# gnovack/distributed-training-and-deepspeed

Hardware: AMD Instinct MI355X
Metric: tokens/sec (whole node) BERT-base DDP (higher is better)
Workload: dtype bf16; 1 GPU; model=bert-base-cased, params=108340804, global_batch=1024, per_gpu_batch=1024, seq_len=512, parallelism=dp1, grad_dtype=bfloat16, impl=fused, mlm_head=sparse (labelled rows only, static capacity 80896; identical loss/grads), optimizer=fused AdamW (transformers.AdamW hyper-params, lr 5e-5), tuned_gemms=True, hip_graph=False, force_collectives=False, prewarm=auto, async_wgrad=False, opt_overlap=True

## Files before the change

distributed_training_and_deepspeed_amd/ops/csrc/attention.hip:

```cpp
#include <stdio.h>
#include <type_traits>
#include <stdlib.h>
#include <string.h>

#include "common.h"

#ifndef DTD_ATTN_FUSED_BWD
#define DTD_ATTN_FUSED_BWD 0
#endif

using namespace dtd;

typedef float f32x16 __attribute__((ext_vector_type(16)));

namespace {

constexpr float kLog2e = 1.4426950408889634f;
constexpr float kLn2 = 0.6931471805599453f;

typedef short s16x4 __attribute__((ext_vector_type(4)));
typedef __attribute__((address_space(3))) s16x4 lds_s16x4;

__device__ __forceinline__ f32x16 mfma32(bf16x8 a, bf16x8 b, f32x16 c) {
  return __builtin_amdgcn_mfma_f32_32x32x16_bf16(a, b, c, 0, 0, 0);
// ... 37 lines not shown
}
__device__ __forceinline__ float keep_bits(float v, uint32_t w, int b) {
  return __int_as_float(__float_as_int(v) & bit_mask(w, b));
}

__device__ __forceinline__ float xhalf_max(float x) {
  const auto r = __builtin_amdgcn_permlane32_swap(__float_as_uint(x), __float_as_uint(x), false, false);
  return fmaxf(__uint_as_float(r[0]), __uint_as_float(r[1]));
}
__device__ __forceinline__ float xhalf_sum(float x) {
  const auto r = __builtin_amdgcn_permlane32_swap(__float_as_uint(x), __float_as_uint(x), false, false);
  return __uint_as_float(r[0]) + __uint_as_float(r[1]);
}
__device__ __forceinline__ uint32_t half_word(uint32_t w, int hh) { return w >> (4 * hh); }
constexpr float kRescaleThr = 8.f;

typedef float f32x2 __attribute__((ext_vector_type(2)));
__device__ __forceinline__ f32x2 pk_fma(f32x2 a, f32x2 b, f32x2 c) { return __builtin_elementwise_fma(a, b, c); }
__device__ __forceinline__ f32x2 pk2(float x, float y) { return f32x2{x, y}; }
__device__ __forceinline__ float mask_bits(float v, int m) { return __int_as_float(__float_as_int(v) & m); }

__device__ __forceinline__ int lm_pos(int x) {
  const int c = x & 31;
  return (x & ~31) | (c & 24) | ((c & 3) << 1) | ((c >> 2) & 1);
}
__device__ __forceinline__ float sel_keep(float v, uint64_t m) {
  float r;
  asm("v_cndmask_b32_e64 %0, 0, %1, %2" : "=v"(r) : "v"(v), "s"(m));
  return r;
}
typedef __attribute__((address_space(4))) const uint64_t cu64;
__device__ __forceinline__ int keep_off(int off, int Sp) { return min(off, Sp - 32); }

struct FwdArgs {
  const bf16* q; const bf16* k; const bf16* v; bf16* o; float* lse; const float* slopes;
  const uint32_t* maskA;
  const uint32_t* maskB;
  int B, S, H, ld, ldo, causal, W;
  float scale, p, thr;
  const int* kv_range;
};

__device__ __forceinline__ void load_range(const int* kv_range, int b, int S, int& lo, int& hi) {
  lo = __builtin_amdgcn_readfirstlane(min(max(kv_range[2 * b], 0), S));
  hi = __builtin_amdgcn_readfirstlane(max(min(kv_range[2 * b + 1], S), 0));
}

template <int S_>
__device__ __forceinline__ uint32_t swap_stage(uint32_t t, uint32_t sh, uint32_t mk) {
  const uint32_t y = (uint32_t)__builtin_amdgcn_ds_swizzle((int)t, (S_ << 10) | 0x1f);
  const uint32_t rot = __builtin_amdgcn_alignbit(y, y, sh);
  return (rot & mk) | (t & ~mk);
}
constexpr int kMaskRot = 13;
__global__ void __launch_bounds__(256) attn_mask_kernel(uint32_t* __restrict__ maskA, uint32_t* __restrict__ maskB,
                                                        int S, int W, const uint64_t* rng, uint32_t sid, uint32_t thr) {
  const int lane = threadIdx.x & 63, bh = blockIdx.y;
  const int q0 = blockIdx.x * 256 + (threadIdx.x & ~63);
  if (q0 >= 32 * W) return;
  DropoutRng g(rng, sid);
  const int q = q0 + lane;
  const bool qv = q < S;
  uint32_t st[16];
  {
    uint32_t x = g.bits((uint64_t)bh * S + (uint64_t)(qv ? q : 0));
    x = x ? x : 0x6d2b79f5u;
#pragma unroll
    for (int i = 0; i < 16; ++i) {
      if (i) { x ^= x << 13; x ^= x >> 17; x ^= x << 5; }
      st[i] = x;
    }
  }
  uint32_t nt[16];
#pragma unroll
  for (int i = 0; i < 16; ++i) nt[i] = ((thr >> i) & 1u) ? 0u : 0xffffffffu;
  const uint32_t live = (qv && thr < 65536u) ? 0xffffffffu : 0u;
  uint32_t sh[5], mk[5];
#pragma unroll
  for (int i = 0; i < 5; ++i) {
    const int s = 16 >> i;
    const uint32_t Hs = i == 0 ? 0xffff0000u : i == 1 ? 0xff00ff00u : i == 2 ? 0xf0f0f0f0u : i == 3 ? 0xccccccccu : 0xaaaaaaaau;
    const bool up = lane & s;
    sh[i] = up ? s : 32 - s;
    mk[i] = up ? ~Hs : Hs;
  }
  const int qw = q0 / 32 + (lane >> 5);
  uint32_t* pa = maskA + (size_t)bh * W * (32 * W) + lm_pos(q);
  for (int kw = 0; kw < W; ++kw) {
    uint32_t acc = 0xffffffffu;
#pragma unroll
    for (int i = 0; i < 16; ++i) {
      st[i] += __builtin_amdgcn_alignbit(st[(i + 11) & 15], st[(i + 11) & 15], 32 - kMaskRot);
      acc = __builtin_amdgcn_bitop3_b32(st[i], acc, nt[i], 0xe8);
    }
    uint32_t word = acc & live;
    const int nk = S - kw * 32;
    if (nk < 32) word &= (0xffffffffu >> (32 - nk));
    if (qv) pa[(size_t)kw * (32 * W)] = word;
    uint32_t t = word;
    t = swap_stage<16>(t, sh[0], mk[0]);
    t = swap_stage<8>(t, sh[1], mk[1]);
    t = swap_stage<4>(t, sh[2], mk[2]);
    t = swap_stage<2>(t, sh[3], mk[3]);
    t = swap_stage<1>(t, sh[4], mk[4]);
    const int key = kw * 32 + (lane & 31);
    if (key < S && qw < W) maskB[((size_t)bh * W + qw) * (32 * W) + lm_pos(key)] = t;
  }
}

__device__ __forceinline__ void xcd_tile(int& tx, int& ty) {
  const int nx = gridDim.x, n = nx * gridDim.y;
  const int L = blockIdx.x + nx * blockIdx.y;
  if (n % 8) { tx = blockIdx.x; ty = blockIdx.y; return; }
  const int T = (L % 8) * (n / 8) + L / 8;
  tx = T % nx;
  ty = T / nx;
}

__device__ __forceinline__ void xcd_tile_grouped(int& tx, int& ty) {
  constexpr int kGroup = 32;
  const int nx = gridDim.x, n = nx * gridDim.y;
  const int L = blockIdx.x + nx * blockIdx.y;
  if (n % 8) { tx = blockIdx.x; ty = blockIdx.y; return; }
  const int per = n / 8, gs = kGroup * nx;
  int i = L / 8;
  if (i < (per / gs) * gs) {
    const int r = i % gs;
    i = (i - r) + (r % kGroup) * nx + r / kGroup;
  }
  const int T = (L % 8) * per + i;
  tx = T % nx;
  ty = T / nx;
}

__device__ __forceinline__ __amdgpu_buffer_rsrc_t bounded_rsrc(const void* p, uint32_t bytes) {
  const uint64_t a = (uint64_t)p;
  const uint32_t lo = __builtin_amdgcn_readfirstlane((uint32_t)a);
  const uint32_t hi = __builtin_amdgcn_readfirstlane((uint32_t)(a >> 32));
  return __builtin_amdgcn_make_buffer_rsrc((void*)(((uint64_t)hi << 32) | lo), (short)0, (int)bytes, 0x00020000);
}

struct RowSrc {
  __amdgpu_buffer_rsrc_t rs;
  int voff, ld2;
};
template <int D>
__device__ __forceinline__ RowSrc row_src(const bf16* base, int ld, int nrows) {
  RowSrc r;
  r.rs = bounded_rsrc(base, nrows > 0 ? (uint32_t)(((nrows - 1) * ld + D) * 2) : 0u);
  r.voff = ((threadIdx.x / (D / 8)) * ld + (threadIdx.x % (D / 8)) * 8) * 2;
  r.ld2 = ld * 2;
  return r;
}
struct WordSrc {
  __amdgpu_buffer_rsrc_t rs;
  int voff, stride;
  __device__ __forceinline__ uint32_t load(int wi) const {
    return __builtin_amdgcn_raw_buffer_load_b32(rs, voff, wi * stride, 0);
  }
};
__device__ __forceinline__ WordSrc word_src(const uint32_t* words, const void* dummy, int W, int pos) {
  WordSrc w;
  const int Sp = 32 * W;
  w.rs = bounded_rsrc(words ? (const void*)words : dummy, words ? (uint32_t)W * Sp * 4u : 0u);
  w.voff = lm_pos(pos) * 4;
  w.stride = Sp * 4;
  return w;
}

template <int D, int ROWS>
struct TileLoader {
  static constexpr int CH = ROWS * D / 8;
  static constexpr int PER = (CH + 255) / 256;
  static constexpr int RPI = 256 / (D / 8);
  bf16x8 reg[PER];
  static_assert(CH % 256 == 0, "tile must split evenly over 256 threads");
  __device__ __forceinline__ void load(const RowSrc& src, int row0) {
#pragma unroll
    for (int i = 0; i < PER; ++i)
      reg[i] = __builtin_bit_cast(bf16x8, __builtin_amdgcn_raw_buffer_load_b128(src.rs, src.voff, (row0 + RPI * i) * src.ld2, 0));
  }
  __device__ __forceinline__ void store(bf16* lds, int stride) const {
#pragma unroll
    for (int i = 0; i < PER; ++i) {
      const int c = threadIdx.x + 256 * i;
      *reinterpret_cast<bf16x8*>(lds + (c / (D / 8)) * stride + (c % (D / 8)) * 8) = reg[i];
    }
  }
  __device__ __forceinline__ void store_swz(bf16* lds) const {
    static_assert(D == 64, "swizzled tile image is for 64-column tiles");
#pragma unroll
    for (int i = 0; i < PER; ++i) {
      const int c = threadIdx.x + 256 * i;
      *reinterpret_cast<bf16x8*>(lds + swz64_off(c >> 3, c & 7)) = reg[i];
    }
  }
  __device__ __forceinline__ void store_bwd(bf16* lds, int stride) const {
    if constexpr (D == 64) store_swz(lds);
    else store(lds, stride);
  }
};

template <int D, int OCC, int BN, int RING, bool PK = false, bool RANGE = false>
__global__ void __launch_bounds__(256, OCC) attn_fwd_kernel(FwdArgs a) {
  constexpr int KP = D + 8, VP = D + 32, NC = D / 16, NDB = D / 32, NKB = BN / 32;
  __shared__ __attribute__((aligned(16))) bf16 Ks[2][BN * KP];
  __shared__ __attribute__((aligned(16))) bf16 Vs[2][BN * VP];

  const int lane = threadIdx.x & 63, w = __builtin_amdgcn_readfirstlane(threadIdx.x >> 6), hh = lane >> 5,
            r = lane & 31;
  int tx, ty;
  xcd_tile(tx, ty);
  const int bh = ty, b = bh / a.H, h = bh % a.H;
  const int S = a.S;
  const int qblk = tx * 128, q0 = qblk + w * 32;
  const int q = q0 + r;
  const bool qvalid = q < S;
  const float sl2 = a.slopes ? a.slopes[h] * kLog2e : 0.f;
  const float sc2 = a.scale * kLog2e;
  const bool drop = a.maskA != nullptr;
  const float inv_keep = drop ? 1.f / (1.f - a.p) : 1.f;
  const RowSrc ksrc = row_src<D>(a.k + (size_t)b * S * a.ld + h * D, a.ld, S);
  const RowSrc vsrc = row_src<D>(a.v + (size_t)b * S * a.ld + h * D, a.ld, S);
  const int Sp = 32 * a.W;
  const uint32_t* mrow = drop ? a.maskB + ((size_t)bh * a.W + min(q0 >> 5, a.W - 1)) * Sp : nullptr;
  const __amdgpu_buffer_rsrc_t mrs = bounded_rsrc(drop ? (const void*)mrow : (const void*)a.lse, drop ? (uint32_t)Sp * 4u : 0u);

  bf16x8 qf[NC];
  {
    const bf16* qp = a.q + ((size_t)(b * S + (qvalid ? q : 0)) * a.ld + h * D);
#pragma unroll
    for (int c = 0; c < NC; ++c) qf[c] = qvalid ? *reinterpret_cast<const bf16x8*>(qp + 16 * c + 8 * hh) : bf16x8{};
  }
  f32x16 oacc[NDB];
#pragma unroll
  for (int d = 0; d < NDB; ++d) oacc[d] = f32x16{};
  float m = -INFINITY, l = 0.f;

  int klo = 0, khi = S;
  if constexpr (RANGE) load_range(a.kv_range, b, S, klo, khi);
  const int kend = a.causal ? min(khi, qblk + 128) : khi;
  const int nt = (kend + BN - 1) / BN;
  const int t0 = RANGE ? klo / BN : 0;
  const int last = RANGE ? max(nt - 1, t0) : nt - 1;
  TileLoader<D, BN> kl0, vl0, kl1r, vl1r;
  TileLoader<D, BN>& kl1 = RING == 2 ? kl1r : kl0;
  TileLoader<D, BN>& vl1 = RING == 2 ? vl1r : vl0;
  uint32_t pf0 = 0, pf1r = 0;
  uint32_t& pf1 = RING == 2 ? pf1r : pf0;
  auto prefetch_words = [&](int k0, uint32_t& out) {
    asm volatile("" :: "v"(out));
    out = __builtin_amdgcn_raw_buffer_load_b32(mrs, lane * 4, k0 * 4, 0);
  };
  kl0.load(ksrc, t0 * BN);
  vl0.load(vsrc, t0 * BN);
  kl0.store(Ks[0], KP);
  vl0.store(Vs[0], VP);
  {
    const int k1 = min(t0 + 1, last) * BN, k2 = min(t0 + 2, last) * BN;
    kl1.load(ksrc, k1); vl1.load(vsrc, k1); prefetch_words(k1, pf1);
    if constexpr (RING == 2) { kl0.load(ksrc, k2); vl0.load(vsrc, k2); prefetch_words(k2, pf0); }
  }
  __syncthreads();
  auto tile = [&](auto set_c, int t) {
    constexpr int SET = decltype(set_c)::value;
    TileLoader<D, BN>& kn = SET ? kl1 : kl0;
    TileLoader<D, BN>& vn = SET ? vl1 : vl0;
    uint32_t& pfn = SET ? pf1 : pf0;
    const int buf = (t - t0) & 1, k0 = t * BN;
    const bf16* K = Ks[buf];
    const bf16* V = Vs[buf];
    uint64_t mk[16];
    auto load_masks = [&](int kb) {
      const cu64* mp = (const cu64*)(uintptr_t)(mrow + keep_off(k0 + kb * 32, Sp));
#pragma unroll
      for (int i = 0; i < 16; ++i) mk[i] = mp[i];
    };
    f32x16 sacc[NKB];
#pragma unroll
    for (int kb = 0; kb < NKB; ++kb) {
      f32x16 acc = f32x16{};
#pragma unroll
      for (int c = 0; c < NC; ++c)
        acc = mfma32(*reinterpret_cast<const bf16x8*>(&K[(kb * 32 + r) * KP + 16 * c + 8 * hh]), qf[c], acc);
      sacc[kb] = acc;
    }
    if (drop) load_masks(0);
    const bool needmask = (k0 + BN > khi) || (RANGE && k0 < klo) || (a.causal && k0 + BN - 1 > q0);
    const bool slow = needmask || sl2 != 0.f;
    float tmax = -INFINITY;
    if (slow) {
#pragma unroll
      for (int kb = 0; kb < NKB; ++kb)
#pragma unroll
        for (int i = 0; i < 16; ++i) {
          const int key = k0 + kb * 32 + crow(i, hh);
          float s = fmaf(sacc[kb][i], sc2, sl2 * (float)key);
          if (needmask && (key >= khi || (RANGE && key < klo) || (a.causal && key > q))) s = -INFINITY;
          sacc[kb][i] = s;
          tmax = fmaxf(tmax, s);
        }
    } else {
#pragma unroll
      for (int kb = 0; kb < NKB; ++kb)
#pragma unroll
        for (int i = 0; i < 16; ++i) tmax = fmaxf(tmax, sacc[kb][i]);
// ... 173 lines not shown
#pragma unroll
        for (int i = 0; i < 16; ++i) tmax = fmaxf(tmax, cur[kb][i]);
      tmax *= sc2;
    }
    tmax = xhalf_max(tmax);
    if (!__all(tmax - m <= a.thr)) {
      const float mnew = fmaxf(m, tmax);
      const float alpha = m == -INFINITY ? 0.f : fexp2(m - mnew);
      m = mnew;
      l *= alpha;
#pragma unroll
      for (int d = 0; d < NDB; ++d) oacc[d] *= alpha;
    }
    scores_kb(Knext, nxt, 1);
    const float mexp = m == -INFINITY ? 0.f : m;
    const float msc = slow ? 1.f : sc2;
    float ps[4];
#pragma unroll
    for (int kb = 0; kb < NKB; ++kb)
#pragma unroll
      for (int i = 0; i < 16; ++i) {
        const float pv = fexp2(fmaf(cur[kb][i], msc, -mexp));
        ps[i & 3] = (kb == 0 && i < 4) ? pv : ps[i & 3] + pv;
        cur[kb][i] = pv;
      }
    l += (ps[0] + ps[1]) + (ps[2] + ps[3]);
    if (drop) {
#pragma unroll
      for (int kb = 0; kb < NKB; ++kb) {
        const uint32_t mw = half_word(mwc[kb], hh);
#pragma unroll
        for (int i = 0; i < 16; ++i) cur[kb][i] = keep_bits(cur[kb][i], mw, crow(i, 0));
      }
    }
#pragma unroll
    for (int kb = 0; kb < NKB; ++kb)
#pragma unroll
      for (int s2 = 0; s2 < 2; ++s2) {
        bf16x8 pf;
#pragma unroll
        for (int j = 0; j < 8; ++j) pf[j] = (bf16)cur[kb][8 * s2 + j];
#pragma unroll
        for (int d = 0; d < NDB; ++d) oacc[d] = mfma32(tr_operand(V, VP, kb * 32 + 16 * s2, d * 32, lane), pf, oacc[d]);
      }
    if (t + 1 < nt) {
      if (t + 2 < nt) kl.store(Ks[t & 1], KP);
      vl.store(Vs[(t + 1) & 1], VP);
#pragma unroll
      for (int j = 0; j < NKB; ++j) mwc[j] = mwn[j];
      kl.load(ksrc, min(t + 3, last) * BN);
      vl.load(vsrc, min(t + 2, last) * BN);
      load_words(min(t + 2, last) * BN, mwn);
    }
    __syncthreads();
  };
  f32x16 sA[NKB], sB[NKB];
#pragma unroll
  for (int kb = 0; kb < NKB; ++kb) scores_kb(Ks[0], sA, kb);
  for (int t = 0; t < nt; t += 2) {
    tile_step(sA, sB, Ks[1], t);
    if (t + 1 < nt) tile_step(sB, sA, Ks[0], t + 1);
  }
  l = xhalf_sum(l);
  if (!qvalid) return;
  const float inv_l = l > 0.f ? inv_keep / l : 0.f;
  bf16* op = a.o + (size_t)(b * S + q) * a.ldo + h * D;
#pragma unroll
  for (int d = 0; d < NDB; ++d)
#pragma unroll
    for (int gq = 0; gq < 4; ++gq) {
      bf16x4 v4;
#pragma unroll
      for (int t = 0; t < 4; ++t) v4[t] = (bf16)(oacc[d][4 * gq + t] * inv_l);
      *reinterpret_cast<bf16x4*>(op + d * 32 + 8 * gq + 4 * hh) = v4;
    }
  if (hh == 0) a.lse[(size_t)bh * S + q] = (m + log2f(l)) * kLn2;
}

struct BwdArgs {
  const bf16* q; const bf16* k; const bf16* v; const bf16* dout; const float* lse; float* delta;
  const bf16* o;
  bf16* dq; bf16* dk; bf16* dv; const float* slopes;
  const uint32_t* maskA; const uint32_t* maskB;
  int B, S, H, ld, ldo, causal, W;
  float scale, p;
  float* bias_part;
  const int* kv_range;
};

template <int S_>
__device__ __forceinline__ float xswz(float x) {
  return __int_as_float(__builtin_amdgcn_ds_swizzle(__float_as_int(x), (S_ << 10) | 0x1f));
}
template <int S_, int N>
__device__ __forceinline__ void rs_step(const float (&in)[2 * N], float (&out)[N], int r) {
  const bool hi = (r & S_) != 0;
#pragma unroll
  for (int j = 0; j < N; ++j) {
    const float mine = hi ? in[j + N] : in[j];
    const float other = hi ? in[j] : in[j + N];
    out[j] = mine + xswz<S_>(other);
  }
}
__device__ __forceinline__ float colsum32(const float (&v)[32], int r) {
  float a16[16], a8[8], a4[4], a2[2], a1[1];
  rs_step<16, 16>(v, a16, r);
  rs_step<8, 8>(a16, a8, r);
  rs_step<4, 4>(a8, a4, r);
  rs_step<2, 2>(a4, a2, r);
  rs_step<1, 1>(a2, a1, r);
  return a1[0];
}
__device__ __forceinline__ int colsum_col(int k, int hh) { return (k >> 4) * 32 + crow(k & 15, hh); }

template <int D, int OCC, int BM, bool DROP, bool ALIBI, bool MASK = true, bool RANGE = false>
__global__ void __launch_bounds__(256, OCC) attn_bwd_dkdv_kernel(BwdArgs a) {
  static_assert(MASK || !RANGE, "a key range needs the masked form");
  constexpr bool SWZ = D == 64;
  constexpr int QP = SWZ ? D : D + 8, NC = D / 16, NDB = D / 32;
  struct Smem {
    float lse_s[2][BM], del_s[2][BM];
    bf16 Qs[2][BM * QP];
    bf16 Os[2][BM * QP];
  };
  __shared__ __attribute__((aligned(16))) Smem sm;
  auto& lse_s = sm.lse_s;
  auto& del_s = sm.del_s;
  auto& Qs = sm.Qs;
  auto& Os = sm.Os;

  const int lane = threadIdx.x & 63, w = __builtin_amdgcn_readfirstlane(threadIdx.x >> 6), hh = lane >> 5,
            r = lane & 31;
  int tx, ty;
  if constexpr (RANGE) xcd_tile_grouped(tx, ty);
  else xcd_tile(tx, ty);
  const int bh = ty, b = bh / a.H, h = bh % a.H;
  const int S = a.S;
  const int kblk = tx * 128;
  const int key = kblk + w * 32 + r;
  const bool kvalid = key < S;
  int klo = 0, khi = S;
  if constexpr (RANGE) {
    load_range(a.kv_range, b, S, klo, khi);
    if (kblk >= khi || kblk + 128 <= klo) {
      if (a.bias_part && D == 64) {
        float* row = a.bias_part + ((size_t)b * gridDim.x * 4 + (kblk >> 5) + w) * (3 * a.H * D) + h * D + colsum_col(r, hh);
        row[a.H * D] = 0.f;
        row[2 * a.H * D] = 0.f;
      }
      if (kvalid) {
        bf16* dkp = a.dk + (size_t)(b * S + key) * a.ld + h * D;
        bf16* dvp = a.dv + (size_t)(b * S + key) * a.ld + h * D;
#pragma unroll
        for (int c = 0; c < D / 8; ++c) {
          *reinterpret_cast<bf16x4*>(dkp + 8 * c + 4 * hh) = bf16x4{};
          *reinterpret_cast<bf16x4*>(dvp + 8 * c + 4 * hh) = bf16x4{};
        }
      }
      return;
    }
  }
  const bool kin = key >= klo && key < khi;
  const float sl2 = a.slopes ? a.slopes[h] * kLog2e : 0.f;
  const float sc2 = a.scale * kLog2e;
  constexpr bool drop = DROP;
  const float inv_keep = drop ? 1.f / (1.f - a.p) : 1.f;
  const float kbias = sl2 * (float)key;
  const int Sp = 32 * a.W;
  const uint32_t* mrow = drop ? a.maskA + ((size_t)bh * a.W + min((kblk >> 5) + w, a.W - 1)) * Sp : nullptr;
  const __amdgpu_buffer_rsrc_t mrs = bounded_rsrc(drop ? (const void*)mrow : (const void*)a.lse, drop ? (uint32_t)Sp * 4u : 0u);
  const RowSrc qsrc = row_src<D>(a.q + (size_t)b * S * a.ld + h * D, a.ld, S);
  const RowSrc osrc = row_src<D>(a.dout + (size_t)b * S * a.ldo + h * D, a.ldo, S);
  const float* lseb = a.lse + (size_t)bh * S;
  const float* delb = a.delta + (size_t)bh * S;

  bf16x8 kf[NC], vf[NC];
  {
    const size_t off = (size_t)(b * S + (kvalid ? key : 0)) * a.ld + h * D;
#pragma unroll
    for (int c = 0; c < NC; ++c) {
      kf[c] = kvalid ? *reinterpret_cast<const bf16x8*>(a.k + off + 16 * c + 8 * hh) : bf16x8{};
      vf[c] = kvalid ? *reinterpret_cast<const bf16x8*>(a.v + off + 16 * c + 8 * hh) : bf16x8{};
    }
  }
  f32x16 dk[NDB], dv[NDB];
#pragma unroll
  for (int d = 0; d < NDB; ++d) { dk[d] = f32x16{}; dv[d] = f32x16{}; }

  const int qstart = a.causal ? (kblk / BM) * BM : 0;
  const int nt = (S - qstart + BM - 1) / BM;
  TileLoader<D, BM> ql, ol;
  float lse_r = 0.f, del_r = 0.f;
  auto load_stats = [&](int q0) {
    if (threadIdx.x < BM) {
      const int qq = q0 + threadIdx.x;
      lse_r = qq < S ? -lseb[qq] * kLog2e : 0.f;
      if constexpr (RANGE) lse_r = lse_r == INFINITY ? -INFINITY : lse_r;
      del_r = qq < S ? -delb[qq] * (DROP ? 1.f - a.p : 1.f) : 0.f;
    }
  };
  constexpr int NPF = BM / 64;
  uint32_t pfw[NPF] = {};
  auto prefetch_words = [&](int q0) {
#pragma unroll
    for (int j = 0; j < NPF; ++j) {
      asm volatile("" :: "v"(pfw[j]));
      pfw[j] = __builtin_amdgcn_raw_buffer_load_b32(mrs, (lane + 64 * j) * 4, q0 * 4, 0);
    }
  };
  ql.load(qsrc, qstart);
  ol.load(osrc, qstart);
  load_stats(qstart);
  ql.store_bwd(Qs[0], QP);
  ol.store_bwd(Os[0], QP);
  if (threadIdx.x < BM) { lse_s[0][threadIdx.x] = lse_r; del_s[0][threadIdx.x] = del_r; }
  __syncthreads();
  for (int t = 0; t < nt; ++t) {
    const int buf = t & 1, q0 = qstart + t * BM;
    if (t + 1 < nt) {
      ql.load(qsrc, q0 + BM);
      ol.load(osrc, q0 + BM);
      load_stats(q0 + BM);
      if (drop) prefetch_words(q0 + BM);
    }
    const bf16* Q = Qs[buf];
    const bf16* O = Os[buf];
    constexpr int kQbUnroll = OCC == 1 ? BM / 32 : 1;
#pragma unroll kQbUnroll
    for (int qb = 0; qb < BM / 32; ++qb) {
      f32x16 sacc = f32x16{}, pacc = f32x16{};
#pragma unroll
      for (int c = 0; c < NC; ++c) {
        if constexpr (SWZ) {
          sacc = mfma32(swz_row_read(Q, qb * 32, r, 2 * c + hh), kf[c], sacc);
          pacc = mfma32(swz_row_read(O, qb * 32, r, 2 * c + hh), vf[c], pacc);
        } else {
          sacc = mfma32(*reinterpret_cast<const bf16x8*>(&Q[(qb * 32 + r) * QP + 16 * c + 8 * hh]), kf[c], sacc);
          pacc = mfma32(*reinterpret_cast<const bf16x8*>(&O[(qb * 32 + r) * QP + 16 * c + 8 * hh]), vf[c], pacc);
        }
      }
      const int qrow0 = q0 + qb * 32;
      bool needmask = MASK && ((kblk + 128 > S) || (qrow0 + 32 > S) || (a.causal && kblk + 127 > qrow0));
      if constexpr (RANGE) needmask = needmask || kblk + 128 > khi || kblk < klo;
      uint64_t mk[16];
      if constexpr (DROP) {
        const cu64* mp = (const cu64*)(uintptr_t)(mrow + keep_off(qrow0, Sp));
#pragma unroll
        for (int i = 0; i < 16; ++i) mk[i] = mp[i];
      }
      f32x4 L4[4], D4[4];
#pragma unroll
      for (int g = 0; g < 4; ++g) {
        L4[g] = *reinterpret_cast<const f32x4*>(&lse_s[buf][qb * 32 + 8 * g + 4 * hh]);
        D4[g] = *reinterpret_cast<const f32x4*>(&del_s[buf][qb * 32 + 8 * g + 4 * hh]);
      }
      const f32x2 sc2v = pk2(sc2, sc2), kb2 = pk2(kbias, kbias);
#pragma unroll
      for (int i = 0; i < 16; i += 2) {
        f32x2 nl = pk2(L4[i >> 2][i & 3], L4[i >> 2][(i & 3) + 1]);
        if constexpr (ALIBI) nl += kb2;
        const f32x2 x = pk_fma(pk2(sacc[i], sacc[i + 1]), sc2v, nl);
        sacc[i] = fexp2(x.x);
        sacc[i + 1] = fexp2(x.y);
      }
      if (MASK && needmask) {
#pragma unroll
        for (int i = 0; i < 16; ++i) {
          const int qq = qrow0 + crow(i, hh);
          bool ok = kvalid && qq < S && !(a.causal && key > qq);
          if constexpr (RANGE) ok = ok && kin;
          sacc[i] = ok ? sacc[i] : 0.f;
        }
      }
#pragma unroll
      for (int i = 0; i < 16; i += 2) {
        const f32x2 nd = pk2(D4[i >> 2][i & 3], D4[i >> 2][(i & 3) + 1]);
        if constexpr (DROP) {
          const f32x2 pm = pk2(sel_keep(sacc[i], mk[i]), sel_keep(sacc[i + 1], mk[i + 1]));
          const f32x2 u = pk2(sacc[i], sacc[i + 1]) * nd;
          const f32x2 ds = pk_fma(pm, pk2(pacc[i], pacc[i + 1]), u);
          pacc[i] = ds.x;
          pacc[i + 1] = ds.y;
          sacc[i] = pm.x;
          sacc[i + 1] = pm.y;
        } else {
          const f32x2 ds = pk2(sacc[i], sacc[i + 1]) * (pk2(pacc[i], pacc[i + 1]) + nd);
          pacc[i] = ds.x;
          pacc[i + 1] = ds.y;
        }
      }
#pragma unroll
      for (int s = 0; s < 2; ++s) {
        bf16x8 pb, sb;
#pragma unroll
        for (int j = 0; j < 8; ++j) { pb[j] = (bf16)sacc[8 * s + j]; sb[j] = (bf16)pacc[8 * s + j]; }
#pragma unroll
        for (int d = 0; d < NDB; ++d) {
          if constexpr (SWZ) {
            dv[d] = mfma32(tr_operand_swz(O, qb * 32 + 16 * s, d * 32, lane), pb, dv[d]);
            dk[d] = mfma32(tr_operand_swz(Q, qb * 32 + 16 * s, d * 32, lane), sb, dk[d]);
          } else {
            dv[d] = mfma32(tr_operand(O, QP, qb * 32 + 16 * s, d * 32, lane), pb, dv[d]);
            dk[d] = mfma32(tr_operand(Q, QP, qb * 32 + 16 * s, d * 32, lane), sb, dk[d]);
          }
        }
      }
    }
    if (t + 1 < nt) {
      ql.store_bwd(Qs[buf ^ 1], QP);
      ol.store_bwd(Os[buf ^ 1], QP);
      if (threadIdx.x < BM) { lse_s[buf ^ 1][threadIdx.x] = lse_r; del_s[buf ^ 1][threadIdx.x] = del_r; }
    }
    __syncthreads();
  }
  const float dv_scale = inv_keep;
  const float dk_scale = a.scale * inv_keep;
  if (a.bias_part && D == 64) {
    float vk[32], vv[32];
#pragma unroll
    for (int d = 0; d < NDB; ++d)
#pragma unroll
      for (int i = 0; i < 16; ++i) {
        vk[16 * d + i] = kvalid ? (float)(bf16)(dk[d][i] * dk_scale) : 0.f;
        vv[16 * d + i] = kvalid ? (float)(bf16)(dv[d][i] * dv_scale) : 0.f;
      }
    const float sk = colsum32(vk, r), sv = colsum32(vv, r);
    float* row = a.bias_part + ((size_t)b * gridDim.x * 4 + (kblk >> 5) + w) * (3 * a.H * D) + h * D + colsum_col(r, hh);
    row[a.H * D] = sk;
    row[2 * a.H * D] = sv;
  }
  if (!kvalid) return;
  bf16* dkp = a.dk + (size_t)(b * S + key) * a.ld + h * D;
  bf16* dvp = a.dv + (size_t)(b * S + key) * a.ld + h * D;
#pragma unroll
  for (int d = 0; d < NDB; ++d)
#pragma unroll
    for (int gq = 0; gq < 4; ++gq) {
      bf16x4 k4, v4;
#pragma unroll
      for (int t = 0; t < 4; ++t) { k4[t] = (bf16)(dk[d][4 * gq + t] * dk_scale); v4[t] = (bf16)(dv[d][4 * gq + t] * dv_scale); }
      *reinterpret_cast<bf16x4*>(dkp + d * 32 + 8 * gq + 4 * hh) = k4;
      *reinterpret_cast<bf16x4*>(dvp + d * 32 + 8 * gq + 4 * hh) = v4;
    }
}

template <int D, int OCC, int BN, int RING, bool PK = false, bool RANGE = false>
__global__ void __launch_bounds__(256, OCC) attn_bwd_dq_kernel(BwdArgs a) {
  constexpr bool SWZ = D == 64;
  constexpr int KP = SWZ ? D : D + 8, NC = D / 16, NDB = D / 32;
  __shared__ __attribute__((aligned(16))) bf16 Ks[2][BN * KP];
  __shared__ __attribute__((aligned(16))) bf16 Vs[2][BN * KP];

  const int lane = threadIdx.x & 63, w = __builtin_amdgcn_readfirstlane(threadIdx.x >> 6), hh = lane >> 5,
            r = lane & 31;
  int tx, ty;
  xcd_tile(tx, ty);
  const int bh = ty, b = bh / a.H, h = bh % a.H;
  const int S = a.S;
  const int qblk = tx * 128, q0 = qblk + w * 32;
  const int q = q0 + r;
  const bool qvalid = q < S;
  const float sl2 = a.slopes ? a.slopes[h] * kLog2e : 0.f;
  const float sc2 = a.scale * kLog2e;
  const bool drop = a.maskA != nullptr;
  const float inv_keep = drop ? 1.f / (1.f - a.p) : 1.f;
  const RowSrc ksrc = row_src<D>(a.k + (size_t)b * S * a.ld + h * D, a.ld, S);
  const RowSrc vsrc = row_src<D>(a.v + (size_t)b * S * a.ld + h * D, a.ld, S);
  const int Sp = 32 * a.W;
  const uint32_t* mrow = drop ? a.maskB + ((size_t)bh * a.W + min(q0 >> 5, a.W - 1)) * Sp : nullptr;
  const __amdgpu_buffer_rsrc_t mrs = bounded_rsrc(drop ? (const void*)mrow : (const void*)a.lse, drop ? (uint32_t)Sp * 4u : 0u);

  bf16x8 qf[NC], of[NC];
  {
    const bf16* qp = a.q + ((size_t)(b * S + (qvalid ? q : 0)) * a.ld + h * D);
    const bf16* op = a.dout + ((size_t)(b * S + (qvalid ? q : 0)) * a.ldo + h * D);
#pragma unroll
    for (int c = 0; c < NC; ++c) {
      qf[c] = qvalid ? *reinterpret_cast<const bf16x8*>(qp + 16 * c + 8 * hh) : bf16x8{};
      of[c] = qvalid ? *reinterpret_cast<const bf16x8*>(op + 16 * c + 8 * hh) : bf16x8{};
    }
  }
  float lse2 = qvalid ? a.lse[(size_t)bh * S + q] * kLog2e : 0.f;
  if constexpr (RANGE) lse2 = lse2 == -INFINITY ? INFINITY : lse2;
  float dl;
  {
    const bf16* orow = a.o + ((size_t)(b * S + (qvalid ? q : 0)) * a.ldo + h * D);
    float part = 0.f;
#pragma unroll
    for (int c = 0; c < NC; ++c) {
      const bf16x8 ov = qvalid ? *reinterpret_cast<const bf16x8*>(orow + 16 * c + 8 * hh) : bf16x8{};
#pragma unroll
      for (int j = 0; j < 8; ++j) part = fmaf((float)ov[j], (float)of[c][j], part);
    }
    dl = xhalf_sum(part);
    if (qvalid && hh == 0) a.delta[(size_t)bh * S + q] = dl;
  }
  f32x16 dq[NDB];
#pragma unroll
  for (int d = 0; d < NDB; ++d) dq[d] = f32x16{};

  int klo = 0, khi = S;
  if constexpr (RANGE) load_range(a.kv_range, b, S, klo, khi);
  const int kend = a.causal ? min(khi, qblk + 128) : khi;
  const int nt = (kend + BN - 1) / BN;
  const int t0 = RANGE ? klo / BN : 0;
  const int last = RANGE ? max(nt - 1, t0) : nt - 1;
  constexpr int NKB = BN / 32;
  TileLoader<D, BN> kl0, vl0, kl1r, vl1r;
  TileLoader<D, BN>& kl1 = RING == 2 ? kl1r : kl0;
  TileLoader<D, BN>& vl1 = RING == 2 ? vl1r : vl0;
  uint32_t pf0 = 0, pf1r = 0;
  uint32_t& pf1 = RING == 2 ? pf1r : pf0;
  auto prefetch_words = [&](int k0, uint32_t& out) {
    asm volatile("" :: "v"(out));
    out = __builtin_amdgcn_raw_buffer_load_b32(mrs, lane * 4, k0 * 4, 0);
  };
  kl0.load(ksrc, t0 * BN);
  vl0.load(vsrc, t0 * BN);
  kl0.store_bwd(Ks[0], KP);
  vl0.store_bwd(Vs[0], KP);
  {
    const int k1 = min(t0 + 1, last) * BN, k2 = min(t0 + 2, last) * BN;
    kl1.load(ksrc, k1); vl1.load(vsrc, k1); prefetch_words(k1, pf1);
    if constexpr (RING == 2) { kl0.load(ksrc, k2); vl0.load(vsrc, k2); prefetch_words(k2, pf0); }
  }
  __syncthreads();
  auto tile = [&](auto set_c, int t) {
    constexpr int SET = decltype(set_c)::value;
    TileLoader<D, BN>& kn = SET ? kl1 : kl0;
    TileLoader<D, BN>& vn = SET ? vl1 : vl0;
    uint32_t& pfn = SET ? pf1 : pf0;
    const int buf = (t - t0) & 1, k0 = t * BN;
    const bf16* K = Ks[buf];
    const bf16* V = Vs[buf];
    const bool needmask = !qvalid || (k0 + BN > khi) || (RANGE && k0 < klo) || (a.causal && k0 + BN - 1 > q0);
#pragma unroll
    for (int kb = 0; kb < BN / 32; ++kb) {
      f32x16 sacc = f32x16{}, pacc = f32x16{};
#pragma unroll
      for (int c = 0; c < NC; ++c) {
        if constexpr (SWZ) {
          sacc = mfma32(swz_row_read(K, kb * 32, r, 2 * c + hh), qf[c], sacc);
          pacc = mfma32(swz_row_read(V, kb * 32, r, 2 * c + hh), of[c], pacc);
        } else {
          sacc = mfma32(*reinterpret_cast<const bf16x8*>(&K[(kb * 32 + r) * KP + 16 * c + 8 * hh]), qf[c], sacc);
          pacc = mfma32(*reinterpret_cast<const bf16x8*>(&V[(kb * 32 + r) * KP + 16 * c + 8 * hh]), of[c], pacc);
        }
      }
      uint64_t mk[16];
      if (drop) {
        const cu64* mp = (const cu64*)(uintptr_t)(mrow + keep_off(k0 + kb * 32, Sp));
#pragma unroll
        for (int i = 0; i < 16; ++i) mk[i] = mp[i];
      }
      if (needmask || sl2 != 0.f) {
#pragma unroll
        for (int i = 0; i < 16; ++i) {
          const int key = k0 + kb * 32 + crow(i, hh);
          float pv = fexp2(fmaf(sacc[i], sc2, sl2 * (float)key - lse2));
          if (needmask && (!qvalid || key >= khi || (RANGE && key < klo) || (a.causal && key > q))) pv = 0.f;
          sacc[i] = pv;
        }
      } else if constexpr (PK) {
        const f32x2 sc22 = pk2(sc2, sc2), nl2 = pk2(-lse2, -lse2);
#pragma unroll
        for (int i = 0; i < 16; i += 2) {
          const f32x2 x = pk_fma(pk2(sacc[i], sacc[i + 1]), sc22, nl2);
          sacc[i] = fexp2(x.x);
          sacc[i + 1] = fexp2(x.y);
        }
      } else {
#pragma unroll
        for (int i = 0; i < 16; ++i) sacc[i] = fexp2(fmaf(sacc[i], sc2, -lse2));
      }
      if constexpr (PK) {
        const f32x2 ik2 = pk2(drop ? inv_keep : 1.f, drop ? inv_keep : 1.f), nd2 = pk2(-dl, -dl);
#pragma unroll
        for (int i = 0; i < 16; i += 2) {
          f32x2 dp = pk2(pacc[i], pacc[i + 1]);
          if (drop) dp = pk2(sel_keep(pacc[i], mk[i]), sel_keep(pacc[i + 1], mk[i + 1]));
          const f32x2 ds = pk2(sacc[i], sacc[i + 1]) * pk_fma(dp, ik2, nd2);
          sacc[i] = ds.x;
          sacc[i + 1] = ds.y;
        }
      } else if (drop) {
#pragma unroll
        for (int i = 0; i < 16; ++i) sacc[i] *= fmaf(sel_keep(pacc[i], mk[i]), inv_keep, -dl);
      } else {
#pragma unroll
        for (int i = 0; i < 16; ++i) sacc[i] *= pacc[i] - dl;
      }
#pragma unroll
      for (int s = 0; s < 2; ++s) {
        bf16x8 sb;
#pragma unroll
        for (int j = 0; j < 8; ++j) sb[j] = (bf16)sacc[8 * s + j];
#pragma unroll
        for (int d = 0; d < NDB; ++d) {
          if constexpr (SWZ) dq[d] = mfma32(tr_operand_swz(K, kb * 32 + 16 * s, d * 32, lane), sb, dq[d]);
          else dq[d] = mfma32(tr_operand(K, KP, kb * 32 + 16 * s, d * 32, lane), sb, dq[d]);
        }
      }
    }
    if (t + 1 < nt) {
      kn.store_bwd(Ks[buf ^ 1], KP);
      vn.store_bwd(Vs[buf ^ 1], KP);
      const int kf = min(t + 1 + RING, nt - 1) * BN;
      kn.load(ksrc, kf);
      vn.load(vsrc, kf);
      prefetch_words(kf, pfn);
    }
    __syncthreads();
  };
  for (int t = t0; t < nt; t += 2) {
    tile(std::integral_constant<int, 1>{}, t);
    if (t + 1 < nt) tile(std::integral_constant<int, 0>{}, t + 1);
  }
  if (a.bias_part && D == 64) {
    float vq[32];
#pragma unroll
    for (int d = 0; d < NDB; ++d)
#pragma unroll
      for (int i = 0; i < 16; ++i) vq[16 * d + i] = qvalid ? (float)(bf16)(dq[d][i] * a.scale) : 0.f;
    const float sq = colsum32(vq, r);
    a.bias_part[((size_t)b * gridDim.x * 4 + (qblk >> 5) + w) * (3 * a.H * D) + h * D + colsum_col(r, hh)] = sq;
  }
  if (!qvalid) return;
  bf16* qp = a.dq + (size_t)(b * S + q) * a.ld + h * D;
#pragma unroll
  for (int d = 0; d < NDB; ++d)
#pragma unroll
    for (int gq = 0; gq < 4; ++gq) {
      bf16x4 v4;
#pragma unroll
      for (int t = 0; t < 4; ++t) v4[t] = (bf16)(dq[d][4 * gq + t] * a.scale);
      *reinterpret_cast<bf16x4*>(qp + d * 32 + 8 * gq + 4 * hh) = v4;
    }
}

#if DTD_ATTN_FUSED_BWD
__device__ __forceinline__ f32x4 mfma16(bf16x8 a, bf16x8 b, f32x4 c) {
  return __builtin_amdgcn_mfma_f32_16x16x32_bf16(a, b, c, 0, 0, 0);
}

__device__ __forceinline__ void mfma32_a(f32x16& acc, bf16x8 a, bf16x8 b) {
  asm volatile("s_nop 1\n\tv_mfma_f32_32x32x16_bf16 %0, %1, %2, %0" : "+a"(acc) : "v"(a), "v"(b));
}

__device__ __forceinline__ void mfma32_v0(f32x16& acc, bf16x8 a, bf16x8 b) {
  asm volatile("s_nop 1\n\tv_mfma_f32_32x32x16_bf16 %0, %1, %2, 0" : "=&v"(acc) : "v"(a), "v"(b));
}
__device__ __forceinline__ void mfma32_v(f32x16& acc, bf16x8 a, bf16x8 b) {
  asm volatile("s_nop 1\n\tv_mfma_f32_32x32x16_bf16 %0, %1, %2, %0" : "+v"(acc) : "v"(a), "v"(b));
}
__device__ __forceinline__ void mfma_vgpr_wait(f32x16& x, f32x16& y) {
  asm volatile("s_nop 11" : "+v"(x), "+v"(y));
}
__device__ __forceinline__ void mfma16_v(f32x4& acc, bf16x8 a, bf16x8 b) {
  asm volatile("s_nop 1\n\tv_mfma_f32_16x16x32_bf16 %0, %1, %2, %0" : "+v"(acc) : "v"(a), "v"(b));
}

template <int NKB, bool DROP>
__global__ void __launch_bounds__(256, 1) attn_bwd_fused_kernel(BwdArgs a) {
  constexpr int D = 64, NC = 4, NDB = 2, SK = 128 * NKB, KPW = 32 * NKB, NT = SK / 32;
  constexpr int KH = NKB % 2 == 0 ? 2 : 1, NH = NKB / KH;
  constexpr int DSP = 36;
  constexpr int DSR = 4 * KH * 32;
  struct Smem {
    float lse_s[32], del_s[32];
    bf16 Qs[32 * 64];
    bf16 Os[32 * 64];
    bf16 DS[DSR * DSP];
    bf16 Ks[SK * 64];
    bf16 Vs[SK * 64];
  };
  __shared__ __attribute__((aligned(16))) Smem sm;

  const int tid = threadIdx.x, lane = tid & 63, w = __builtin_amdgcn_readfirstlane(tid >> 6), hh = lane >> 5,
            r = lane & 31;
  const int bh = blockIdx.x, b = bh / a.H, h = bh % a.H;
  const int S = a.S;
  const float sc2 = a.scale * kLog2e;
  const float inv_keep = DROP ? 1.f / (1.f - a.p) : 1.f;
  const int kw0 = w * KPW;
  const int Sp = 32 * a.W;
  const float* lseb = a.lse + (size_t)bh * S;
  const RowSrc qsrc = row_src<D>(a.q + (size_t)b * S * a.ld + h * D, a.ld, S);
  const RowSrc dsrc = row_src<D>(a.dout + (size_t)b * S * a.ldo + h * D, a.ldo, S);
  const RowSrc osrc = row_src<D>(a.o + (size_t)b * S * a.ldo + h * D, a.ldo, S);
  {
    const RowSrc ksrc = row_src<D>(a.k + (size_t)b * S * a.ld + h * D, a.ld, S);
    const RowSrc vsrc = row_src<D>(a.v + (size_t)b * S * a.ld + h * D, a.ld, S);
#pragma unroll
    for (int half = 0; half < 2; ++half) {
      TileLoader<D, SK / 2> kl, vl;
      kl.load(ksrc, half * (SK / 2));
      vl.load(vsrc, half * (SK / 2));
      kl.store_swz(sm.Ks + half * (SK / 2) * 64);
      vl.store_swz(sm.Vs + half * (SK / 2) * 64);
    }
  }
  TileLoader<D, 32> ql, dl, ol;
  float lse_n = 0.f;
  auto fetch = [&](int q0) {
    ql.load(qsrc, q0);
    dl.load(dsrc, q0);
    ol.load(osrc, q0);
    if (tid < 32) lse_n = lseb[q0 + tid];
  };
  auto stage = [&]() {
    float part = 0.f;
#pragma unroll
    for (int j = 0; j < 8; ++j) part = fmaf((float)dl.reg[0][j], (float)ol.reg[0][j], part);
    part += __shfl_xor(part, 1, 64);
    part += __shfl_xor(part, 2, 64);
    part += __shfl_xor(part, 4, 64);
    ql.store_swz(sm.Qs);
    dl.store_swz(sm.Os);
    if ((tid & 7) == 0) sm.del_s[tid >> 3] = -part;
    if (tid < 32) sm.lse_s[tid] = -lse_n * kLog2e;
  };
  fetch(0);
  stage();

  f32x16 dk[NKB][NDB], dv[NKB][NDB];
#pragma unroll
  for (int kb = 0; kb < NKB; ++kb)
#pragma unroll
    for (int d = 0; d < NDB; ++d) { dk[kb][d] = f32x16{}; dv[kb][d] = f32x16{}; }
  const int g16 = lane >> 4, l16 = lane & 15, qq = l16 >> 2, pp = l16 & 3;
  const int kcol = 16 * w + 4 * pp;
  __syncthreads();

  for (int t = 0; t < NT; ++t) {
    const int q0 = t * 32;
    if (t + 1 < NT) fetch(q0 + 32);
    f32x4 dq2[2] = {f32x4{}, f32x4{}};
#pragma unroll
    for (int hf = 0; hf < NH; ++hf) {
#pragma unroll
      for (int kk = 0; kk < KH; ++kk) {
        const int kb = hf * KH + kk;
        const int key0 = kw0 + 32 * kb;
        f32x16 sacc, pacc;
#pragma unroll
        for (int c = 0; c < NC; ++c) {
          const bf16x8 qa = swz_row_read(sm.Qs, 0, r, 2 * c + hh), kr = swz_row_read(sm.Ks, key0, r, 2 * c + hh);
          const bf16x8 oa = swz_row_read(sm.Os, 0, r, 2 * c + hh), vr = swz_row_read(sm.Vs, key0, r, 2 * c + hh);
          if (c == 0) { mfma32_v0(sacc, qa, kr); mfma32_v0(pacc, oa, vr); }
          else { mfma32_v(sacc, qa, kr); mfma32_v(pacc, oa, vr); }
        }
        mfma_vgpr_wait(sacc, pacc);
        uint64_t mk[16];
        if constexpr (DROP) {
          const cu64* mp = (const cu64*)(uintptr_t)(a.maskA + ((size_t)bh * a.W + min(w * NKB + kb, a.W - 1)) * Sp +
                                                    keep_off(q0, Sp));
#pragma unroll
          for (int i = 0; i < 16; ++i) mk[i] = mp[i];
        }
        f32x4 L4[4];
#pragma unroll
        for (int g = 0; g < 4; ++g) L4[g] = *reinterpret_cast<const f32x4*>(&sm.lse_s[8 * g + 4 * hh]);
        const f32x2 sc2v = pk2(sc2, sc2);
#pragma unroll
        for (int i = 0; i < 16; i += 2) {
          const f32x2 x = pk_fma(pk2(sacc[i], sacc[i + 1]), sc2v, pk2(L4[i >> 2][i & 3], L4[i >> 2][(i & 3) + 1]));
          sacc[i] = fexp2(x.x);
          sacc[i + 1] = fexp2(x.y);
        }
        f32x4 D4[4];
#pragma unroll
        for (int g = 0; g < 4; ++g) D4[g] = *reinterpret_cast<const f32x4*>(&sm.del_s[8 * g + 4 * hh]);
#pragma unroll
        for (int i = 0; i < 16; i += 2) {
          const f32x2 nd = pk2(D4[i >> 2][i & 3], D4[i >> 2][(i & 3) + 1]);
          if constexpr (DROP) {
            const f32x2 tt = pk_fma(pk2(sel_keep(pacc[i], mk[i]), sel_keep(pacc[i + 1], mk[i + 1])),
                                    pk2(inv_keep, inv_keep), nd);
            const f32x2 ds = pk2(sacc[i], sacc[i + 1]) * tt;
            pacc[i] = ds.x;
            pacc[i + 1] = ds.y;
            sacc[i] = sel_keep(sacc[i], mk[i]);
            sacc[i + 1] = sel_keep(sacc[i + 1], mk[i + 1]);
          } else {
            const f32x2 ds = pk2(sacc[i], sacc[i + 1]) * (pk2(pacc[i], pacc[i + 1]) + nd);
            pacc[i] = ds.x;
            pacc[i + 1] = ds.y;
          }
        }
        bf16* dsrow = sm.DS + ((w * KH + kk) * 32 + r) * DSP + 4 * hh;
// ... 560 lines not shown
```

Before: 1.464 million tokens/s.

## Widen attention backward stores and overlap dQ-kernel prologue loads with K/V prefetch

Replaces the 8-byte per-lane bf16x4 output stores of dK, dV and dQ with 16-byte stores, using permlane32 swaps so each lane holds 8 contiguous bf16 values. Fragment and stat loads switch to bounded buffer loads, which removes the per-lane validity branches. In the dQ kernel the Q, dO and O fragment loads and the delta computation move so they are issued alongside the first K/V tile loads, hiding their latency. This adds cross-lane swap instructions and more live registers in the prologue, which could lower occupancy.

```diff
diff --git a/distributed_training_and_deepspeed_amd/ops/csrc/attention.hip b/distributed_training_and_deepspeed_amd/ops/csrc/attention.hip
--- a/distributed_training_and_deepspeed_amd/ops/csrc/attention.hip
+++ b/distributed_training_and_deepspeed_amd/ops/csrc/attention.hip
@@ -213,6 +213,43 @@
   r.ld2 = ld * 2;
   return r;
 }
+template <int D>
+__device__ __forceinline__ void load_frags(bf16x8 (&f)[D / 16], const bf16* base, int ld, int nrows, int row, int hh) {
+  const __amdgpu_buffer_rsrc_t rs = bounded_rsrc(base, nrows > 0 ? (uint32_t)(((nrows - 1) * ld + D) * 2) : 0u);
+  const int voff = (row * ld + 8 * hh) * 2;
+#pragma unroll
+  for (int c = 0; c < D / 16; ++c) f[c] = __builtin_bit_cast(bf16x8, __builtin_amdgcn_raw_buffer_load_b128(rs, voff + 32 * c, 0, 0));
+}
+__device__ __forceinline__ float load_stat(__amdgpu_buffer_rsrc_t rs, int off) {
+  return __uint_as_float(__builtin_amdgcn_raw_buffer_load_b32(rs, off, 0, 0));
+}
+
+typedef uint32_t u32x2 __attribute__((ext_vector_type(2)));
+typedef uint32_t u32x4 __attribute__((ext_vector_type(4)));
+template <int NDB>
+__device__ __forceinline__ void store_rows16(bf16* rowp, const f32x16 (&acc)[NDB], float scale, int hh, bool valid) {
+  u32x4 out[2 * NDB];
+#pragma unroll
+  for (int d = 0; d < NDB; ++d)
+#pragma unroll
+    for (int g2 = 0; g2 < 2; ++g2) {
+      bf16x4 a4, b4;
+#pragma unroll
+      for (int t = 0; t < 4; ++t) { a4[t] = (bf16)(acc[d][8 * g2 + t] * scale); b4[t] = (bf16)(acc[d][8 * g2 + 4 + t] * scale); }
+      u32x2 a = __builtin_bit_cast(u32x2, a4), b = __builtin_bit_cast(u32x2, b4);
+#pragma unroll
+      for (int t = 0; t < 2; ++t) {
+        const auto s = __builtin_amdgcn_permlane32_swap(a[t], b[t], false, false);
+        a[t] = s[0];
+        b[t] = s[1];
+      }
+      out[2 * d + g2] = u32x4{a[0], a[1], b[0], b[1]};
+    }
+  if (!valid) return;
+#pragma unroll
+  for (int i = 0; i < 2 * NDB; ++i) *reinterpret_cast<u32x4*>(rowp + 16 * i + 8 * hh) = out[i];
+}
+
 struct WordSrc {
   __amdgpu_buffer_rsrc_t rs;
   int voff, stride;
@@ -692,9 +729,9 @@
         bf16* dkp = a.dk + (size_t)(b * S + key) * a.ld + h * D;
         bf16* dvp = a.dv + (size_t)(b * S + key) * a.ld + h * D;
 #pragma unroll
-        for (int c = 0; c < D / 8; ++c) {
-          *reinterpret_cast<bf16x4*>(dkp + 8 * c + 4 * hh) = bf16x4{};
-          *reinterpret_cast<bf16x4*>(dvp + 8 * c + 4 * hh) = bf16x4{};
+        for (int c = 0; c < D / 16; ++c) {
+          *reinterpret_cast<bf16x8*>(dkp + 16 * c + 8 * hh) = bf16x8{};
+          *reinterpret_cast<bf16x8*>(dvp + 16 * c + 8 * hh) = bf16x8{};
         }
       }
       return;
@@ -711,18 +748,12 @@
   const __amdgpu_buffer_rsrc_t mrs = bounded_rsrc(drop ? (const void*)mrow : (const void*)a.lse, drop ? (uint32_t)Sp * 4u : 0u);
   const RowSrc qsrc = row_src<D>(a.q + (size_t)b * S * a.ld + h * D, a.ld, S);
   const RowSrc osrc = row_src<D>(a.dout + (size_t)b * S * a.ldo + h * D, a.ldo, S);
-  const float* lseb = a.lse + (size_t)bh * S;
-  const float* delb = a.delta + (size_t)bh * S;
+  const __amdgpu_buffer_rsrc_t lse_rs = bounded_rsrc(a.lse + (size_t)bh * S, (uint32_t)S * 4u);
+  const __amdgpu_buffer_rsrc_t del_rs = bounded_rsrc(a.delta + (size_t)bh * S, (uint32_t)S * 4u);
 
   bf16x8 kf[NC], vf[NC];
-  {
-    const size_t off = (size_t)(b * S + (kvalid ? key : 0)) * a.ld + h * D;
-#pragma unroll
-    for (int c = 0; c < NC; ++c) {
-      kf[c] = kvalid ? *reinterpret_cast<const bf16x8*>(a.k + off + 16 * c + 8 * hh) : bf16x8{};
-      vf[c] = kvalid ? *reinterpret_cast<const bf16x8*>(a.v + off + 16 * c + 8 * hh) : bf16x8{};
-    }
-  }
+  load_frags<D>(kf, a.k + (size_t)b * S * a.ld + h * D, a.ld, S, key, hh);
+  load_frags<D>(vf, a.v + (size_t)b * S * a.ld + h * D, a.ld, S, key, hh);
   f32x16 dk[NDB], dv[NDB];
 #pragma unroll
   for (int d = 0; d < NDB; ++d) { dk[d] = f32x16{}; dv[d] = f32x16{}; }
@@ -731,12 +762,18 @@
   const int nt = (S - qstart + BM - 1) / BM;
   TileLoader<D, BM> ql, ol;
   float lse_r = 0.f, del_r = 0.f;
+  const int stat_off = threadIdx.x < BM ? (int)threadIdx.x * 4 : 0x40000000;
   auto load_stats = [&](int q0) {
+    lse_r = load_stat(lse_rs, q0 * 4 + stat_off);
+    del_r = load_stat(del_rs, q0 * 4 + stat_off);
+  };
+  auto store_stats = [&](int buf, int q0) {
     if (threadIdx.x < BM) {
-      const int qq = q0 + threadIdx.x;
-      lse_r = qq < S ? -lseb[qq] * kLog2e : 0.f;
-      if constexpr (RANGE) lse_r = lse_r == INFINITY ? -INFINITY : lse_r;
-      del_r = qq < S ? -delb[qq] * (DROP ? 1.f - a.p : 1.f) : 0.f;
+      const bool in = q0 + (int)threadIdx.x < S;
+      float nl = in ? -lse_r * kLog2e : 0.f;
+      if constexpr (RANGE) nl = nl == INFINITY ? -INFINITY : nl;
+      lse_s[buf][threadIdx.x] = nl;
+      del_s[buf][threadIdx.x] = in ? -del_r * (DROP ? 1.f - a.p : 1.f) : 0.f;
     }
   };
   constexpr int NPF = BM / 64;
@@ -753,7 +790,7 @@
   load_stats(qstart);
   ql.store_bwd(Qs[0], QP);
   ol.store_bwd(Os[0], QP);
-  if (threadIdx.x < BM) { lse_s[0][threadIdx.x] = lse_r; del_s[0][threadIdx.x] = del_r; }
+  store_stats(0, qstart);
   __syncthreads();
   for (int t = 0; t < nt; ++t) {
     const int buf = t & 1, q0 = qstart + t * BM;
@@ -849,7 +886,7 @@
     if (t + 1 < nt) {
       ql.store_bwd(Qs[buf ^ 1], QP);
       ol.store_bwd(Os[buf ^ 1], QP);
-      if (threadIdx.x < BM) { lse_s[buf ^ 1][threadIdx.x] = lse_r; del_s[buf ^ 1][threadIdx.x] = del_r; }
+      store_stats(buf ^ 1, q0 + BM);
     }
     __syncthreads();
   }
@@ -869,19 +906,8 @@
     row[a.H * D] = sk;
     row[2 * a.H * D] = sv;
   }
-  if (!kvalid) return;
-  bf16* dkp = a.dk + (size_t)(b * S + key) * a.ld + h * D;
-  bf16* dvp = a.dv + (size_t)(b * S + key) * a.ld + h * D;
-#pragma unroll
-  for (int d = 0; d < NDB; ++d)
-#pragma unroll
-    for (int gq = 0; gq < 4; ++gq) {
-      bf16x4 k4, v4;
-#pragma unroll
-      for (int t = 0; t < 4; ++t) { k4[t] = (bf16)(dk[d][4 * gq + t] * dk_scale); v4[t] = (bf16)(dv[d][4 * gq + t] * dv_scale); }
-      *reinterpret_cast<bf16x4*>(dkp + d * 32 + 8 * gq + 4 * hh) = k4;
-      *reinterpret_cast<bf16x4*>(dvp + d * 32 + 8 * gq + 4 * hh) = v4;
-    }
+  store_rows16<NDB>(a.dk + (size_t)(b * S + key) * a.ld + h * D, dk, dk_scale, hh, kvalid);
+  store_rows16<NDB>(a.dv + (size_t)(b * S + key) * a.ld + h * D, dv, dv_scale, hh, kvalid);
 }
 
 template <int D, int OCC, int BN, int RING, bool PK = false, bool RANGE = false>
@@ -910,31 +936,6 @@
   const uint32_t* mrow = drop ? a.maskB + ((size_t)bh * a.W + min(q0 >> 5, a.W - 1)) * Sp : nullptr;
   const __amdgpu_buffer_rsrc_t mrs = bounded_rsrc(drop ? (const void*)mrow : (const void*)a.lse, drop ? (uint32_t)Sp * 4u : 0u);
 
-  bf16x8 qf[NC], of[NC];
-  {
-    const bf16* qp = a.q + ((size_t)(b * S + (qvalid ? q : 0)) * a.ld + h * D);
-    const bf16* op = a.dout + ((size_t)(b * S + (qvalid ? q : 0)) * a.ldo + h * D);
-#pragma unroll
-    for (int c = 0; c < NC; ++c) {
-      qf[c] = qvalid ? *reinterpret_cast<const bf16x8*>(qp + 16 * c + 8 * hh) : bf16x8{};
-      of[c] = qvalid ? *reinterpret_cast<const bf16x8*>(op + 16 * c + 8 * hh) : bf16x8{};
-    }
-  }
-  float lse2 = qvalid ? a.lse[(size_t)bh * S + q] * kLog2e : 0.f;
-  if constexpr (RANGE) lse2 = lse2 == -INFINITY ? INFINITY : lse2;
-  float dl;
-  {
-    const bf16* orow = a.o + ((size_t)(b * S + (qvalid ? q : 0)) * a.ldo + h * D);
-    float part = 0.f;
-#pragma unroll
-    for (int c = 0; c < NC; ++c) {
-      const bf16x8 ov = qvalid ? *reinterpret_cast<const bf16x8*>(orow + 16 * c + 8 * hh) : bf16x8{};
-#pragma unroll
-      for (int j = 0; j < 8; ++j) part = fmaf((float)ov[j], (float)of[c][j], part);
-    }
-    dl = xhalf_sum(part);
-    if (qvalid && hh == 0) a.delta[(size_t)bh * S + q] = dl;
-  }
   f32x16 dq[NDB];
 #pragma unroll
   for (int d = 0; d < NDB; ++d) dq[d] = f32x16{};
@@ -955,14 +956,33 @@
     asm volatile("" :: "v"(out));
     out = __builtin_amdgcn_raw_buffer_load_b32(mrs, lane * 4, k0 * 4, 0);
   };
-  kl0.load(ksrc, t0 * BN);
-  vl0.load(vsrc, t0 * BN);
-  kl0.store_bwd(Ks[0], KP);
-  vl0.store_bwd(Vs[0], KP);
+  bf16x8 qf[NC], of[NC];
+  float lse2, dl;
   {
+    TileLoader<D, BN> kpr, vpr;
+    TileLoader<D, BN>& kp = RING == 2 ? kl0 : kpr;
+    TileLoader<D, BN>& vp = RING == 2 ? vl0 : vpr;
     const int k1 = min(t0 + 1, last) * BN, k2 = min(t0 + 2, last) * BN;
+    kp.load(ksrc, t0 * BN);
+    vp.load(vsrc, t0 * BN);
     kl1.load(ksrc, k1); vl1.load(vsrc, k1); prefetch_words(k1, pf1);
+    bf16x8 ov[NC];
+    load_frags<D>(qf, a.q + (size_t)b * S * a.ld + h * D, a.ld, S, q, hh);
+    load_frags<D>(of, a.dout + (size_t)b * S * a.ldo + h * D, a.ldo, S, q, hh);
+    load_frags<D>(ov, a.o + (size_t)b * S * a.ldo + h * D, a.ldo, S, q, hh);
+    lse2 = load_stat(bounded_rsrc(a.lse + (size_t)bh * S, (uint32_t)S * 4u), q * 4) * kLog2e;
+    if constexpr (RANGE) lse2 = lse2 == -INFINITY ? INFINITY : lse2;
+    asm volatile("" ::: "memory");
+    kp.store_bwd(Ks[0], KP);
+    vp.store_bwd(Vs[0], KP);
     if constexpr (RING == 2) { kl0.load(ksrc, k2); vl0.load(vsrc, k2); prefetch_words(k2, pf0); }
+    float part = 0.f;
+#pragma unroll
+    for (int c = 0; c < NC; ++c)
+#pragma unroll
+      for (int j = 0; j < 8; ++j) part = fmaf((float)ov[c][j], (float)of[c][j], part);
+    dl = xhalf_sum(part);
+    if (qvalid && hh == 0) a.delta[(size_t)bh * S + q] = dl;
   }
   __syncthreads();
   auto tile = [&](auto set_c, int t) {
@@ -1065,17 +1085,7 @@
     const float sq = colsum32(vq, r);
     a.bias_part[((size_t)b * gridDim.x * 4 + (qblk >> 5) + w) * (3 * a.H * D) + h * D + colsum_col(r, hh)] = sq;
   }
-  if (!qvalid) return;
-  bf16* qp = a.dq + (size_t)(b * S + q) * a.ld + h * D;
-#pragma unroll
-  for (int d = 0; d < NDB; ++d)
-#pragma unroll
-    for (int gq = 0; gq < 4; ++gq) {
-      bf16x4 v4;
-#pragma unroll
-      for (int t = 0; t < 4; ++t) v4[t] = (bf16)(dq[d][4 * gq + t] * a.scale);
-      *reinterpret_cast<bf16x4*>(qp + d * 32 + 8 * gq + 4 * hh) = v4;
-    }
+  store_rows16<NDB>(a.dq + (size_t)(b * S + q) * a.ld + h * D, dq, a.scale, hh, qvalid);
 }
 
 #if DTD_ATTN_FUSED_BWD
```

After: 1.482 million tokens/s, median of 6. 1.2% higher.
